# pathint/RankCompV3.jl

Hardware: AMD Instinct MI355X
Metric: gene-pair·sample comparisons/sec at 20k genes × 1k samples (higher is better)
Workload: dtype u16

## Files before the change

### rankcompv3.jl_amd/_ffi.py

```python
from __future__ import annotations

import ctypes
import os
import subprocess
from typing import NamedTuple

import numpy as np

_HERE = os.path.dirname(os.path.abspath(__file__))
LIB_PATH = os.environ.get("REO_LIB_PATH") or os.path.join(_HERE, "libreo_hip.so")
CSRC = os.path.join(_HERE, "csrc")

REO_OK, REO_EINVAL, REO_EHIP, REO_ECOMM, REO_ENOMEM = 0, -1, -2, -3, -4
NTIMINGS = 12
CALL_BINS = 8192

SYMBOLS = [
    "reo_version", "reo_last_error", "reo_create", "reo_destroy", "reo_trim_memory", "reo_set_shard", "reo_set_allreduce", "reo_set_allgather",
    "reo_create_multi", "reo_comm_unique_id", "reo_comm_init_rank",
    "reo_set_matrix_f64", "reo_set_matrix_i64", "reo_set_matrix_dev_f64", "reo_set_matrix_dev_i64",
    "reo_set_matrix_f32", "reo_set_matrix_i32", "reo_set_matrix_dev_f32", "reo_set_matrix_dev_i32",
    "reo_set_matrix_rm_f64", "reo_set_matrix_rm_i64", "reo_set_matrix_rm_f32", "reo_set_matrix_rm_i32",
    "reo_set_matrix_csc_f64", "reo_set_matrix_csc_i64", "reo_set_matrix_csc_f32", "reo_set_matrix_csc_i32",
    "reo_set_groups", "reo_compute_thresholds", "reo_set_thresholds", "reo_get_thresholds", "reo_threshold",
# ... 837 lines not shown
    def get_matrix(self) -> np.ndarray:
        info = self.info()
        dt = {1: np.float64, 2: np.int64, 3: np.float32}.get(info["resident_dtype"])
        if dt is None:
            raise DimensionMismatch(REO_EINVAL, "no expression matrix set")
        out = np.zeros((info["G"], info["S"]), dtype=dt, order="F")
        check(self._L.reo_get_matrix(self._h, _ptr(out), out.nbytes))
        return out

    def set_profiling(self, on: bool) -> None:
        check(self._L.reo_set_profiling(self._h, 1 if on else 0))

    def reset_timings(self) -> None:
        check(self._L.reo_reset_timings(self._h))

    def timings(self) -> dict:
        ms = np.zeros(NTIMINGS, dtype=np.float64)
        check(self._L.reo_get_timings(self._h, _ptr(ms), NTIMINGS))
        return {"transform_ms": ms[0], "k1_ms": ms[1], "k2_ms": ms[2], "iter_ms": ms[3], "k3_ms": max(ms[3] - ms[2], 0.0), "k2_launches": int(ms[4]),
                "k1_launches": int(ms[5]), "exchange_ms": ms[6], "pseudobulk_ms": ms[7], "k2_full_ms": ms[8],
                "k2_full_launches": int(ms[9]), "k2_delta_ms": ms[10], "set_matrix_host_wall_ms": ms[11]}

    def info(self) -> dict:
        w = np.zeros(32, dtype=np.int64)
        check(self._L.reo_get_info(self._h, _ptr(w), 32))
        v = np.zeros(28, dtype=np.int64)
        v[:] = w[:28]
        return {"G": int(v[0]), "S": int(v[1]), "Gp": int(v[2]), "table_bytes": int(v[3]), "has_ties": int(v[4]),
                "tiles_owned": int(v[5]), "tiles_total": int(v[6]), "tile_i": int(v[7]), "chunk_j": int(v[8]),
                "chunks_per_panel": int(v[9]), "unit_h": int(v[10]), "sample_slots": int(v[11]),
                "shared_group_counts": int(v[12]), "group_count_bytes": int(v[13]), "transform_in_lds": int(v[14]), "xcc_local_histograms": int(v[15]),
                "cycle_period": int(v[16]), "cycle_found_at_pass": int(v[17]), "cycle_passes_skipped": int(v[18]), "upload_link_bytes": int(v[19]),
                "eager_range_launches": int(v[20]), "rowmajor_upload": int(v[21]),
                "csc_upload": int(v[22]), "csc_nnz": int(v[23]), "resident_dtype": int(v[24]),
                "k1_slot_order": int(v[25]), "k1_half_tiles_separated": int(v[26]), "csc_device": int(v[27]),
                "k1_unslot_form": int(w[28]), "contrast_treat": int(w[29]), "k1_slot_sides": int(w[30]),
                "masked_build": int(w[31])}
```

### rankcompv3.jl_amd/csrc/api.hip

```cpp
#include <execinfo.h>
#include <signal.h>
#include <unistd.h>

#include <ctime>
#include <algorithm>
#include <chrono>
#include <cmath>
#include <cstdarg>
#include <cstdio>
#include <cstdlib>
#include <cstring>

#include "reo_internal.h"
#include "contrast.h"
#include "masked_pairs.h"
#include "sample_counts.h"
#include "upload_csc.h"

#include <mutex>
#include <unordered_map>

namespace reo {

static thread_local std::string g_err;
thread_local bool tl_release_synced = false;

namespace {
struct Block { void *p; size_t bytes; int device; bool pinned; };
struct Pool {
    std::mutex mu;
    std::vector<Block> free_blocks;
    std::unordered_map<void *, size_t> live;
    size_t cached = 0, cap = size_t(16384) << 20;
    bool read_env = false;
};
Pool &pool() { static Pool *p = new Pool(); return *p; }
// ... 569 lines not shown
    }
    REO_HIP_CHECK(hipSetDevice(device));
    reo_ctx *c = new (std::nothrow) reo_ctx();
    if (!c) { set_error("out of host memory"); return REO_ENOMEM; }
    c->device = device;
    c->seed = seed;
    if (const char *e = getenv("REO_K1_WAVE")) c->k1_wave = (e[0] != '0');
    if (const char *e = getenv("REO_K1_HALF")) c->k1_half = (e[0] != '0');
    if (const char *e = getenv("REO_K1_SLOTS")) c->k1_slots = (e[0] != '0');
    if (const char *e = getenv("REO_K1_QUEUE")) c->k1_queue = (e[0] != '0');
    if (const char *e = getenv("REO_K1_UNSLOT")) { const int v = atoi(e); c->k1_unslot = (v == 8 || v == 4) ? v : (e[0] == '0' ? 0 : -1); }
    if (const char *e = getenv("REO_K1_SLOT_SIDES")) { const int v = atoi(e); c->k1_slot_sides = (v == 1 || v == 2) ? v : 0; }
    if (const char *e = getenv("REO_K1_WORKERS")) c->k1_workers = std::max(1, atoi(e));
    if (const char *e = getenv("REO_K1_ORDER")) c->k1_order = std::max(0, std::min(2, atoi(e)));
    {
        int n = 0;
        if (hipDeviceGetAttribute(&n, hipDeviceAttributeMultiprocessorCount, c->device) == hipSuccess && n > 0) c->n_cus = n;
    }
    if (const char *e = getenv("REO_SPIN_WAIT")) c->spin_wait = (e[0] != '0');
    if (const char *e = getenv("REO_CHECK_HOOK_TABLE")) c->check_hook_table = (e[0] != '0');
    if (const char *e = getenv("REO_SHARE_GROUP_COUNTS")) c->share_counts = (e[0] != '0');
    if (const char *e = getenv("REO_LIGHT_BAND")) c->light_band = std::max(0, atoi(e));
    if (const char *e = getenv("REO_HIST_BELOW")) c->hist_below = std::max(0, atoi(e));
    if (const char *e = getenv("REO_CYCLE")) c->cycle_watch = atoi(e) != 0;
    if (const char *e = getenv("REO_LIGHT")) c->light_mode = e[0] == '0' ? 0 : (e[0] == '2' ? 2 : (e[0] == '3' ? 3 : 1));
    c->light_window = light_window(); c->light_min_g = light_min_genes();
    if (const char *e = getenv("REO_LIGHT_WINDOW")) c->light_window = std::max(1, std::min(31, atoi(e)));
    if (const char *e = getenv("REO_LIGHT_MIN_G")) c->light_min_g = std::max(64, atoi(e));
    if (const char *e = getenv("REO_STATE_MIRROR")) c->state_mirror_wanted = (e[0] != '0');
    if (const char *e = getenv("REO_EXCHANGE_WAVES")) c->x_waves = std::max(1, std::min(8, atoi(e)));
    if (const char *e = getenv("REO_EAGER_UPLOAD")) c->eager_mode = std::max(0, std::min(2, atoi(e)));
    if (const char *e = getenv("REO_EAGER_CHUNK")) c->eager_chunk = std::max(1, atoi(e));
    if (const char *e = getenv("REO_EAGER_GATE")) c->eager_gate = atoi(e) != 0;
    if (const char *e = getenv("REO_EAGER_RANGES")) c->eager_ranges = std::max(1, std::min(6, atoi(e)));
    if (const char *e = getenv("REO_UPLOAD_THREADS")) c->upload_threads = std::max(0, std::min(64, atoi(e)));
    c->debug_passes = getenv("REO_DEBUG_PASSES") != nullptr;
    c->debug_stamps = getenv("REO_DEBUG_STAMPS") != nullptr;
    c->k1_stamps = getenv("REO_K1_STAMPS") != nullptr;
    hipError_t e = handle_stream(&c->stream, 0);
    if (e != hipSuccess) { delete c; set_error("hipStreamCreate failed: %s", hipGetErrorString(e)); return REO_EHIP; }
    int ok = 0;
    const char *xe = getenv("REO_XCC_LOCAL");
    if (!(xe && xe[0] == '0')) {
        const int32_t rc = xcc_selftest(c, &ok);
        if (rc) { reo_destroy(c); return rc; }
    }
// ... 823 lines not shown
{
    if (!c) { set_error("null context"); return REO_EINVAL; }
    collect_timings(c);
    for (double &v : c->t_ms) v = 0.0;
    return REO_OK;
}

int32_t reo_get_timings(reo_ctx *c, double *ms, int32_t n)
{
    if (!c || !ms) { set_error("null argument"); return REO_EINVAL; }
    collect_timings(c);
    for (int i = 0; i < n && i < REO_NTIMINGS; ++i) ms[i] = c->t_ms[i];
    return REO_OK;
}

int32_t reo_get_info(reo_ctx *c, int64_t *info, int32_t n)
{
    if (!c || !info) { set_error("null argument"); return REO_EINVAL; }
    int64_t separated = 0;
    if (n > 26 && c->last_k1_slots) {
        int32_t rc = use(c);
        if (rc || (rc = launch_slot_separated(c, &separated))) return rc;
    }
    const int64_t v[32] = {c->G, c->S, c->Gp, static_cast<int64_t>(c->table.n * sizeof(uint32_t)), c->has_ties,
                           c->tiles_owned, c->tiles_total, kTileI, c->k1_cj, c->k1_q, kUnitH,
                           c->goff32.empty() ? 0 : c->goff32.back(), c->last_k1_shared,
                           static_cast<int64_t>(c->gcounts.n * sizeof(uint16_t)), c->transform_in_lds, c->xcc_local,
                           c->it_cycle_period, c->it_cycle_at, c->it_cycle_skipped, c->narrowed_bytes, c->eager_range_launches, c->rowmajor_upload,
                           c->csc_upload, c->csc_nnz, c->dtype, c->last_k1_slots, separated, c->csc_device,
                           c->last_k1_slots ? c->last_k1_unslot : 0, c->built_k >= 0 ? c->built_treat : -1,
                           c->last_k1_slots ? c->last_k1_slot_sides : 0, (c->built_k >= 0 && c->built_masked) ? 1 : 0};
    for (int i = 0; i < n && i < 32; ++i) info[i] = v[i];
    return REO_OK;
}

}
```

### rankcompv3.jl_amd/csrc/kernels.hip

```cpp
#include <algorithm>
#include <chrono>
#include <cstddef>
#include <cstdio>
#include <cstdlib>
#include <cstring>
#include <mutex>
#include <type_traits>

#include "reo_internal.h"
#include "k1_items.h"
#include "k1_slots.h"
#include "k1_queue.h"
#include "contrast.h"
#include "tie_coin.h"

namespace reo {

namespace {

template <bool COH, class T>
__device__ __forceinline__ T ldc(const T *p)
{
    if (COH) return __hip_atomic_load(p, __ATOMIC_RELAXED, __HIP_MEMORY_SCOPE_AGENT);
    return *p;
}
template <bool COH, class T>
__device__ __forceinline__ void stc(T *p, T v)
{
    if (COH) __hip_atomic_store(p, v, __ATOMIC_RELAXED, __HIP_MEMORY_SCOPE_AGENT);
    else *p = v;
}

// ... 1501 lines not shown
    int G, Gp, Wp;
    int n_iter, n_conv;
    int a0, b0;
    double pval_deg, padj_deg;
    uint32_t *refbits[2];
    uint8_t *refbytes[2];
    int32_t *raw;
    uint32_t *delta_list;
    double *result;
    double *chunk_v; uint16_t *chunk_i; double *chunk_spl;
    double *sorted_d; double *sorted_spl; double *sorted_p;
    uint32_t *rank_s; uint32_t *rank_a;
    double *part; double *blockmin; double *scal;
    int32_t *trace; int32_t *modes;
    double *cand;
    int32_t *hist;
    int hist_stride;
    int32_t *mrank;
    int replay;
    int k2_idx;
    int xcc_local;
    int32_t *olist;
    int hist_below;
    uint8_t *snap;
    int32_t *clist; int band;
    int window, light_min_g;
    unsigned long long *stamps;
    IterState *host_st;
};

#ifdef REO_STAMPS
#define STAMP(a, k) do { if (blockIdx.x == 0 && threadIdx.x == 0) (a).stamps[k] = __builtin_amdgcn_s_memrealtime(); } while (0)
#else
#define STAMP(a, k) do { } while (0)
#endif

__device__ __forceinline__ void raise_fault(const IterArgs &a, int code)
{
    a.st->fault = code;
    if (a.host_st) a.host_st->fault = code;
}

constexpr int kCandMax = 64;
constexpr int kWindow = 24;
constexpr int kLightMinG = 4096;

// ... 672 lines not shown
    const double n = n0 + n1 + n2;
    const double mean = (n0 * mean0 + n1 * mean1 + n2 * mean2) / n;
    const double m2 = (q0 + n0 * (mean0 - mean) * (mean0 - mean)) + (q1 + n1 * (mean1 - mean) * (mean1 - mean)) +
                      (q2 + n2 * (mean2 - mean) * (mean2 - mean));
    se = sqrt(m2 / (n - 1.0));
    return static_cast<int>(n) == a.b0 - a.a0 + 1;
}

template <bool COH>
__device__ __forceinline__ bool slice_std(const IterArgs &a, const double *cand, int npart, int below_a, int below_b, int cnt_a, int cnt_b,
                                          double (*sel)[4], double *red, double &se, double &va, double &vb)
{
    const int lane = threadIdx.x & 63, wave = threadIdx.x >> 6;
    double x = 0.0, pn[kPartPer] = {0.0}, pm[kPartPer] = {0.0}, pq[kPartPer] = {0.0};
    if (wave < 2 && lane < (wave ? cnt_b : cnt_a) && lane < kCandMax) x = ldc<COH>(cand + wave * kCandMax + lane);
#pragma unroll
    for (int u = 0; u < kPartPer; ++u) {
        const int w = threadIdx.x + 256 * u;
        if (w < npart) { pn[u] = ldc<COH>(a.part + 3 * w); pm[u] = ldc<COH>(a.part + 3 * w + 1); pq[u] = ldc<COH>(a.part + 3 * w + 2); }
    }
    return slice_std_vals(a, x, pn, pm, pq, below_a, below_b, cnt_a, cnt_b, sel, red, se, va, vb);
}

__device__ __forceinline__ int hist_first(int kstar, int below) { return kstar > below ? kstar - below : 0; }

template <int NT = 4>
__device__ __forceinline__ int bh_cut4(const int (&hv)[4][8], int G, int tile0, int &carry_io, int roff = 0)
{
    __shared__ __attribute__((aligned(16))) int wsum[4][4];
    __shared__ int wbest[4];
    const int lane = threadIdx.x & 63, wave = threadIdx.x >> 6;
    int s[4], inc[4];
#pragma unroll
    for (int e = 0; e < NT; ++e) {
        s[e] = ((hv[e][0] + hv[e][1]) + (hv[e][2] + hv[e][3])) + ((hv[e][4] + hv[e][5]) + (hv[e][6] + hv[e][7]));
        inc[e] = s[e];
    }
#pragma unroll
    for (int o = 1; o < 64; o <<= 1)
#pragma unroll
        for (int e = 0; e < NT; ++e)
        { const int u = __shfl_up(inc[e], o, 64); if (lane >= o) inc[e] += u; }
    if (lane == 63)
#pragma unroll
        for (int e = 0; e < NT; ++e) wsum[e][wave] = inc[e];
    lds_barrier();
    int best = 0, carry = carry_io;
#pragma unroll
    for (int e = 0; e < NT; ++e) {
        const int4 ws = *reinterpret_cast<const int4 *>(wsum[e]);
        int run = carry + inc[e] - s[e] + (wave > 0 ? ws.x : 0) + (wave > 1 ? ws.y : 0) + (wave > 2 ? ws.z : 0);
        const int r0 = roff + ((tile0 + e) * 256 + threadIdx.x) * 8 + 1;
#pragma unroll
        for (int u = 0; u < 8; ++u) { run += hv[e][u]; if (r0 + u <= G && run >= r0 + u) best = max(best, r0 + u); }
        carry += ws.x + ws.y + ws.z + ws.w;
    }
    carry_io = carry;
#pragma unroll
    for (int o = 32; o > 0; o >>= 1) { const int u = __shfl_xor(best, o, 64); best = u > best ? u : best; }
    if (lane == 0) wbest[wave] = best;
    lds_barrier();
    const int k = max(max(wbest[0], wbest[1]), max(wbest[2], wbest[3]));
    lds_barrier();
    return k;
}

template <int BYTES>
__device__ __forceinline__ void warm_kernargs()
{
    const uint32_t *ka = (const uint32_t *)__builtin_amdgcn_kernarg_segment_ptr();
    uint32_t t[(BYTES + 63) / 64];
#pragma unroll
    for (int q = 0; q < (BYTES + 63) / 64; ++q) t[q] = ka[16 * q];
#pragma unroll
    for (int q = 0; q < (BYTES + 63) / 64; ++q) asm volatile("" ::"s"(t[q]));
}

constexpr int kListPre = 5;
constexpr int kHeadPre = 20;

__device__ __forceinline__ int mrank_slot(int i) { return (i & ~255) + 4 * (i & 63) + ((i >> 6) & 3); }

__device__ __forceinline__ unsigned xcc_id()
{
    unsigned x;
    asm volatile("s_getreg_b32 %0, hwreg(HW_REG_XCC_ID, 0, 4)" : "=s"(x));
    return x & (kHistParts - 1);
// ... 64 lines not shown
    const bool crowded = reload_all || __ballot(nflag > 1) != 0;
    if (!crowded && __ballot(nflag == 1)) note_changes(nflag == 1, wave + 4 * selq, sel);
#pragma unroll 1
    for (int R = crowded ? wave : wave + 4 * kHeadPre; R < nrow; R += 4) note_changes(true, R, load_rank_row<COH>(mrank, R, lane));
}

template <bool TAIL, bool LIST>
__global__ __launch_bounds__(256) void kl_head(IterArgs a, LightState *ls, int b)
{
    const int G = a.G, Gp = a.Gp;
    const int i = blockIdx.x * 256 + threadIdx.x;
    const int lane = threadIdx.x & 63, wave = threadIdx.x >> 6;
    __shared__ uint32_t dl[kDeltaMax];
    __shared__ int s_n, s_nn, s_fb;
    __shared__ uint4 dbuf[kDeltaMax * 8];
    __shared__ double red[256];
    warm_kernargs<sizeof(IterArgs) + 16>();
    if (!TAIL) STAMP(a, 8);
    const int pb = (b - 1) & 1;
    LightRec r;
    int bfail = 0, sig = 0, nlow = 0, cdiff = 0, cfound = 0;
    int hv[4][8];
    int4 hx[kHistParts][2];
    int4 mv[kHeadPre];
    int2 le[kListPre];
    int lcnt[kListPre];
    int own_m = 0;
    int4 r0 = make_int4(0, 0, 0, 0), r1 = make_int4(0, 0, 0, 0);
    double win[4];
    uint32_t cyc_w[kDeltaMax / 64];
    uint8_t cyc_s[kDeltaMax / 64];
    int cyc_open = 0;
    bool cyc_renew = false;
    const int nrow = (G + 255) >> 8;
    if (b > 0) {
        const int32_t *hist = a.hist + static_cast<size_t>(pb) * kHistParts * a.hist_stride;
#pragma unroll
        for (int e = 0; e < 4; ++e)
#pragma unroll
            for (int u = 0; u < 8; ++u) hv[e][u] = 0;
#pragma unroll
        for (int x = 0; x < kHistParts; ++x) {
            const int4 *hp = reinterpret_cast<const int4 *>(hist + static_cast<size_t>(x) * a.hist_stride + threadIdx.x * 8);
            hx[x][0] = hp[0]; hx[x][1] = hp[1];
        }
#pragma unroll
        for (int q = 0; q < kHeadPre; ++q) {
            const int R = wave + 4 * q;
            mv[q] = make_int4(0, 0, 0, 0);
            if (!LIST && R < nrow) mv[q] = reinterpret_cast<const int4 *>(a.mrank)[R * 64 + lane];
        }
        if (LIST) {
            const int32_t *cl = a.clist + static_cast<size_t>(pb) * kListStride;
#pragma unroll
            for (int q = 0; q < kListPre; ++q) {
                const int e = threadIdx.x + 256 * q, blk = e / kListCap;
                le[q] = make_int2(0, 0); lcnt[q] = 0;
                if (blk < nrow) { lcnt[q] = cl[blk]; le[q] = reinterpret_cast<const int2 *>(cl + kListWgs)[e]; }
            }
        }
        if (i < G) own_m = a.mrank[mrank_slot(i)];
    }
    if (!TAIL && i < G) {
        const int4 *o = reinterpret_cast<const int4 *>(a.raw + static_cast<size_t>(i) * kRaw);
        r0 = o[0]; r1 = o[1];
    }
    if (b > 0) {
        const LightSlot *ps = &ls->slot[b - 1];
        r = ps->rec; bfail = ps->bfail; cdiff = ps->cdiff; cfound = ps->cfound;
#pragma unroll
        for (int q = 0; q < kSpread; ++q) { sig += ps->lc.sig[q][0]; nlow += ps->lc.nlow[q][0]; }
#pragma unroll
        for (int q = 0; q < 4; ++q) win[q] = ps->wnext[q];
    } else {
#pragma unroll
        for (int q = 0; q < 4; ++q) win[q] = a.scal[1 + q];
    }
    if (!TAIL) STAMP(a, 0);
    int n = 0;
    bool inref = false;
    bool stepped = false;
    if (b == 0) {
        const IterState *st = a.st;
        r.t = st->passes; r.nref = st->nref; r.nref_prev = st->nref_prev; r.done = st->done; r.need_full = st->need_full;
        r.raw_pass = st->raw_pass; r.ran = 0; r.dcnt = st->delta_cnt[r.t & 1]; r.kstar = -1;
        r.cper = st->cyc_period; r.cpow = st->cyc_pow; r.clam = st->cyc_lam; r.csel = st->cyc_sel; cdiff = st->cyc_ndiff;
        r.active = (!r.done && r.t < a.n_iter && !r.need_full) ? 1 : 0;
        if (r.active) {
            n = r.raw_pass == r.t ? 0 : min(r.dcnt, kDeltaMax);
            if (static_cast<int>(threadIdx.x) < n) dl[threadIdx.x] = a.delta_list[static_cast<size_t>(r.t & 1) * Gp + threadIdx.x];
            inref = i < G && a.refbytes[r.t & 1][i] != 0;
            lds_barrier();
        }
    } else if (r.active && bfail) {
        r.active = 0; r.need_full = 1;
    } else if (r.active && cfound) {
        r.active = 0; r.cper = cfound;
    } else if (r.active) {
        const int t = r.t, cur = t & 1, nxt = cur ^ 1;
        const int off = hist_first(r.kstar, a.hist_below), srel = sig - off;
        {
            const int32_t *hist = a.hist + static_cast<size_t>(pb) * kHistParts * a.hist_stride;
#pragma unroll
            for (int x = 0; x < kHistParts; ++x) {
                hv[0][0] += hx[x][0].x; hv[0][1] += hx[x][0].y; hv[0][2] += hx[x][0].z; hv[0][3] += hx[x][0].w;
                hv[0][4] += hx[x][1].x; hv[0][5] += hx[x][1].y; hv[0][6] += hx[x][1].z; hv[0][7] += hx[x][1].w;
            }
            if (srel > 2048) {
#pragma unroll 1
                for (int x = 0; x < kHistParts; ++x)
#pragma unroll
                    for (int e = 1; e < 4; ++e) {
                        const int4 *hp = reinterpret_cast<const int4 *>(hist + static_cast<size_t>(x) * a.hist_stride + (e * 256 + threadIdx.x) * 8);
                        const int4 h0 = hp[0], h1 = hp[1];
                        hv[e][0] += h0.x; hv[e][1] += h0.y; hv[e][2] += h0.z; hv[e][3] += h0.w; hv[e][4] += h1.x; hv[e][5] += h1.y; hv[e][6] += h1.z; hv[e][7] += h1.w;
                    }
            }
        }
        int carry = nlow;
        int kstar = srel > 2048 ? bh_cut4(hv, G, 0, carry, off) : bh_cut4<1>(hv, G, 0, carry, off);
        if (srel > 8192) {
            const int32_t *hist = a.hist + static_cast<size_t>(pb) * kHistParts * a.hist_stride;
            const int ntile = (min(G - off, srel) + 2047) / 2048;
#pragma unroll 1
            for (int tile0 = 4; tile0 < ntile; tile0 += 4) {
#pragma unroll
                for (int e = 0; e < 4; ++e)
#pragma unroll
                    for (int u = 0; u < 8; ++u) hv[e][u] = 0;
#pragma unroll 1
                for (int x = 0; x < kHistParts; ++x)
#pragma unroll
                    for (int e = 0; e < 4; ++e) {
                        if ((tile0 + e) * 2048 >= a.hist_stride) continue;
                        const int4 *hp = reinterpret_cast<const int4 *>(hist + static_cast<size_t>(x) * a.hist_stride + ((tile0 + e) * 256 + threadIdx.x) * 8);
                        const int4 h0 = hp[0], h1 = hp[1];
                        hv[e][0] += h0.x; hv[e][1] += h0.y; hv[e][2] += h0.z; hv[e][3] += h0.w; hv[e][4] += h1.x; hv[e][5] += h1.y; hv[e][6] += h1.z; hv[e][7] += h1.w;
                    }
                kstar = max(kstar, bh_cut4(hv, G, tile0, carry, off));
            }
        }
        const bool cut_lost = off > 0 && kstar == 0;
        if (!TAIL) STAMP(a, 1);
        if (cut_lost) {
            r.active = 0; r.need_full = 1;
        } else {
        if (threadIdx.x == 0) { s_n = 0; s_nn = 0; s_fb = 0; }
        lds_barrier();
        if (LIST) {
            const uint32_t base = static_cast<uint32_t>(kstar) + 1u;
            bool bad = r.kstar < 0 || kstar < r.kstar - a.band || kstar > r.kstar + a.band;
            auto note = [&](int cnt, int2 ent, int e) {
                bad = bad || cnt > kListCap;
                const bool chd = (e % kListCap) < cnt && static_cast<int>(static_cast<uint32_t>(ent.x) - base) >= 0;
                const unsigned long long cm = __ballot(chd);
                if (cm) {
                    const uint32_t nb = (static_cast<uint32_t>(ent.x) >> 31) ^ 1u;
                    const unsigned long long am = __ballot(chd && nb);
                    int pos = 0;
                    if (lane == 0) { pos = atomicAdd(&s_n, __popcll(cm)); atomicAdd(&s_nn, 2 * __popcll(am) - __popcll(cm)); }
                    pos = __shfl(pos, 0, 64);
                    const int at = pos + __popcll(cm & ((1ULL << lane) - 1ULL));
                    if (chd && at < kDeltaMax) dl[at] = (static_cast<uint32_t>(ent.y) << 1) | nb;
                }
            };
#pragma unroll
            for (int q = 0; q < kListPre; ++q) note(lcnt[q], le[q], threadIdx.x + 256 * q);
            const int32_t *cl = a.clist + static_cast<size_t>(pb) * kListStride;
// ... 62 lines not shown
            for (int o = 32; o > 0; o >>= 1) d += __shfl_xor(d, o, 64);
            cdiff += d;
            cfound = cdiff == 0 ? cyc_open : 0;
        } else if (cyc_open < 0) {
            cdiff = 0x40000000; cfound = 0;
        } else {
            cfound = stepped ? 0 : cfound;
        }
        if (cyc_renew) cdiff = 0;
    };
    if (TAIL) {
        if (blockIdx.x == 0 && wave == 0) {
            cyc_close();
            if (cfound) r.cper = cfound;
        }
        if (blockIdx.x == 0 && threadIdx.x == 0) {
            IterState *st = a.st;
            st->cyc_period = r.cper; st->cyc_pow = r.cpow; st->cyc_lam = r.clam; st->cyc_sel = r.csel; st->cyc_ndiff = cdiff;
            st->passes = r.t; st->nref = r.nref; st->nref_prev = r.nref_prev; st->done = r.done; st->need_full = r.need_full;
            st->i_iter = r.t - (r.done ? 1 : 0);
            st->raw_pass = r.raw_pass;
            st->delta_cnt[r.t & 1] = r.dcnt;
            if (r.ran) st->last_full = 0;
            if (stepped) { a.scal[1] = win[0]; a.scal[2] = win[1]; a.scal[3] = win[2]; a.scal[4] = win[3]; }
            if (a.host_st) {
                IterState *h = a.host_st;
                h->passes = r.t; h->done = r.done; h->need_full = r.need_full; h->delta_cnt[r.t & 1] = r.dcnt;
                h->cyc_period = r.cper;
                if (r.ran) h->last_full = 0;
            }
        }
        return;
    }
    if (r.active) r.raw_pass = r.t;
    if (blockIdx.x == 0 && threadIdx.x == 0) ls->slot[b].rec = r;
    if (!r.active || static_cast<int>(blockIdx.x) * 256 >= G) {
        if (blockIdx.x == 0 && wave == 0) { cyc_close(); if (lane == 0) { ls->slot[b].cdiff = cdiff; ls->slot[b].cfound = cfound; } }
        return;
    }
    const int pbuf = b & 1;
    LightCnt *lc = &ls->slot[b].lc;
    const double wa_lo = win[0], wa_hi = win[1], wb_lo = win[2], wb_hi = win[3];
    double v = 0.0;
    bool inner = false, inA = false, inB = false, belowA = false, belowB = false;
    if (n) {
        int d[kRaw];
        delta_counts_block(a.table, a.Wp, dl, n, d, dbuf);
        if (!TAIL) STAMP(a, 3);
        if (i < G) {
            r0.x += d[0]; r0.y += d[1]; r0.z += d[2]; r0.w += d[3];
            r1.x += d[4]; r1.y += d[5]; r1.z += d[6]; r1.w += d[7];
            int4 *o = reinterpret_cast<int4 *>(a.raw + static_cast<size_t>(i) * kRaw);
            o[0] = r0; o[1] = r1;
        }
    }
    if (i < G) {
        int32_t c[9];
        const bool tok = tallies_from(r0, r1, r.nref - (inref ? 1 : 0), c);
        double out[5] = {1.0, 0.0, 0.0, 0.0, 0.0};
        if (tok) mccullagh3<false>(c, out);
        v = out[1];
        if (!tok || !(fabs(v) < INFINITY)) { v = 0.0; raise_fault(a, kFaultTallies); }
        if (!TAIL) STAMP(a, 4);
        a.result[11 * static_cast<size_t>(G) + i] = v;
#pragma unroll
        for (int x = 0; x < kHistParts; ++x) a.hist[(static_cast<size_t>(pbuf) * kHistParts + x) * a.hist_stride + i] = 0;
        belowA = v < wa_lo; inA = !belowA && v <= wa_hi;
        belowB = v < wb_lo; inB = !belowB && v <= wb_hi;
        inner = v > wa_hi && v < wb_lo;
    }
    if (!TAIL) STAMP(a, 5);
    if (G <= 65535) {
        const double nb = static_cast<double>(__popcll(__ballot(inner))), sum = wave_sum(inner ? v : 0.0);
        const double mean = nb > 0.0 ? sum / nb : 0.0;
        const double m2 = wave_sum(inner ? (v - mean) * (v - mean) : 0.0);
        if (lane == 0) { double *pp = a.part + 3 * (4 * blockIdx.x + wave); pp[0] = nb; pp[1] = mean; pp[2] = m2; }
    } else {
        double nb, sum;
        block_sum2_256(inner ? 1.0 : 0.0, inner ? v : 0.0, red, nb, sum);
        const double mean = nb > 0.0 ? sum / nb : 0.0;
        const double m2 = block_sum_256(inner ? (v - mean) * (v - mean) : 0.0, red);
        if (threadIdx.x == 0) { a.part[3 * blockIdx.x] = nb; a.part[3 * blockIdx.x + 1] = mean; a.part[3 * blockIdx.x + 2] = m2; }
    }
    if (!TAIL) STAMP(a, 6);
    const unsigned long long mA = __ballot(inA), mB = __ballot(inB), bA = __ballot(belowA), bB = __ballot(belowB);
    int baseA = 0, baseB = 0;
    if (lane == 0) {
        if (mA) baseA = atomicAdd(&lc->cnt_a, __popcll(mA));
        if (mB) baseB = atomicAdd(&lc->cnt_b, __popcll(mB));
        if (bA) spread_add(lc->below_a, __popcll(bA), a.xcc_local);
        if (bB) spread_add(lc->below_b, __popcll(bB), a.xcc_local);
    }
// ... 31 lines not shown
    const double wd0 = a.scal[5], wd1 = a.scal[6], wd2 = a.scal[7], wd3 = a.scal[8];
    const double d1 = live ? a.result[11 * static_cast<size_t>(G) + i] : 0.0;
    const uint8_t ob_e = live ? a.refbytes[0][i] : 0, ob_o = live ? a.refbytes[1][i] : 0;
    if (!active) return;
    STAMP(a, 20);
    __shared__ double sel[3][4];
    double se = 0.0, va = 0.0, vb = 0.0;
    bool ok = slice_std_split(a, x, pn, pm, pq, below_a, below_b, cnt_a, cnt_b, sel, se, va, vb);
    ok = ok && (va + wd1 < vb - wd2);
    STAMP(a, 21);
    if (blockIdx.x == 0 && threadIdx.x == 0) {
        if (ok) {
            a.scal[0] = se;
            sl->wnext[0] = va - wd0; sl->wnext[1] = va + wd1; sl->wnext[2] = vb - wd2; sl->wnext[3] = vb + wd3;
        } else {
            sl->bfail = 1;
        }
    }
    if (!ok) return;
    const double p = live ? normal_p(d1, se) : 1.0;
    if (live) a.result[i] = p;
    const int m = live ? bh_rank(p, G, a.padj_deg) : G + 1;
    STAMP(a, 22);
    {
        const int off = hist_first(rec_kstar, a.hist_below);
        const unsigned long long first = __ballot(m == 1 && off == 0), finite = __ballot(m <= G), low = __ballot(m <= off);
        const bool lead1 = m == 1 && off == 0 && lane == __ffsll(static_cast<long long>(first)) - 1;
        const bool binned = m > off && m <= G && !(m == 1 && off == 0);
        if (a.xcc_local) {
            int32_t *hist = a.hist + (static_cast<size_t>(pbuf) * kHistParts + xcc_id()) * a.hist_stride;
            if (lead1) __hip_atomic_fetch_add(&hist[0], __popcll(first), __ATOMIC_RELAXED, __HIP_MEMORY_SCOPE_WORKGROUP);
            else if (binned) __hip_atomic_fetch_add(&hist[m - 1 - off], 1, __ATOMIC_RELAXED, __HIP_MEMORY_SCOPE_WORKGROUP);
        } else {
            int32_t *hist = a.hist + static_cast<size_t>(pbuf) * kHistParts * a.hist_stride;
            if (lead1) atomicAdd(&hist[0], __popcll(first));
            else if (binned) atomicAdd(&hist[m - 1 - off], 1);
        }
        if (lane == 0 && finite) spread_add(lc->sig, __popcll(finite), a.xcc_local);
        if (lane == 0 && low) spread_add(lc->nlow, __popcll(low), a.xcc_local);
    }
    {
        __shared__ int32_t row[256];
        const uint32_t oldbit = ((rec_t & 1) ? ob_o : ob_e) != 0 ? 0x80000000u : 0u;
        row[4 * lane + wave] = live ? static_cast<int32_t>(static_cast<uint32_t>(p <= a.pval_deg ? m : G + 2) | oldbit) : 0;
        lds_barrier();
        a.mrank[blockIdx.x * 256 + threadIdx.x] = row[threadIdx.x];
    }
    if (rec_kstar >= 0) {
        __shared__ int s_c;
        if (threadIdx.x == 0) s_c = 0;
        lds_barrier();
        const int kp = rec_kstar, rk = p <= a.pval_deg ? m : G + 2;
        const bool ob = ((rec_t & 1) ? ob_o : ob_e) != 0;
        const bool want = live && ((rk > kp - a.band && rk <= kp + a.band) || (rk > kp + a.band && !ob) || (rk <= kp - a.band && ob));
        const unsigned long long cm = __ballot(want);
        int pos = 0;
        if (cm && lane == 0) pos = atomicAdd(&s_c, __popcll(cm));
        pos = __shfl(pos, 0, 64) + __popcll(cm & ((1ULL << lane) - 1ULL));
        int32_t *cl = a.clist + static_cast<size_t>(pbuf) * kListStride;
        if (want && pos < kListCap)
            reinterpret_cast<int2 *>(cl + kListWgs)[blockIdx.x * kListCap + pos] = make_int2(static_cast<int>(static_cast<uint32_t>(rk) | (ob ? 0x80000000u : 0u)), i);
        lds_barrier();
        if (threadIdx.x == 0) cl[blockIdx.x] = min(s_c, kListCap + 1);
    }
    STAMP(a, 23);
}

constexpr double kEtaMin = 1.0 / 2048.0, kEtaMax = 1.0 / 64.0, kEta0 = 1.0 / 128.0;

// ... 1356 lines not shown
    k3_tallies<<<(G + 255) / 256, 256, 0, c->stream>>>(c->raw.p, c->refbytes[0].p, nref, G, c->cont.p);
    REO_HIP_CHECK(hipGetLastError());
    return REO_OK;
}

static IterArgs iter_args(reo_ctx *c, int replay)
{
    IterArgs a;
    a.st = c->state.p; a.table = c->table.p;
    a.G = static_cast<int>(c->G); a.Gp = c->Gp; a.Wp = c->Wp;
    a.n_iter = c->it_n_iter; a.n_conv = c->it_n_conv; a.a0 = c->it_a0; a.b0 = c->it_b0;
    a.pval_deg = c->it_pval_deg; a.padj_deg = c->it_padj_deg;
    for (int t = 0; t < 2; ++t) { a.refbits[t] = c->refbits[t].p; a.refbytes[t] = c->refbytes[t].p; }
    a.raw = c->raw.p; a.delta_list = c->delta_list.p; a.result = c->result.p;
    const int nchunk = (a.G + kSortChunk - 1) / kSortChunk;
    a.chunk_v = c->chunk_v.p; a.chunk_i = c->chunk_i.p;
    a.chunk_spl = c->chunk_v.p + static_cast<size_t>(nchunk) * kSortChunk;
    a.sorted_d = c->sorted_d.p; a.sorted_spl = c->sorted_d.p + ((c->G + 63) / 64) * 64;
    a.sorted_p = c->sorted_p.p; a.rank_s = c->rank_s.p; a.rank_a = c->rank_a.p;
    a.part = c->part.p; a.blockmin = c->blockmin.p; a.scal = c->scal.p;
    a.trace = c->trace.p; a.modes = nullptr;
    a.cand = c->cand.p; a.hist = c->hist.p; a.hist_stride = static_cast<int>(c->hist.n / (3 * kHistParts)); a.mrank = c->mrank.p;
    a.replay = replay; a.k2_idx = 0;
    a.clist = c->clist.p; a.olist = c->olist.p; a.band = c->light_band; a.hist_below = c->hist_below; a.snap = c->snap.p; a.xcc_local = c->xcc_local;
    a.window = c->light_window; a.light_min_g = (c->it_no_light || c->light_mode == 0) ? 0x7FFFFFFF : c->light_min_g;
    a.stamps = reinterpret_cast<unsigned long long *>(c->scal.p + 32);
    a.host_st = c->state_mirror ? c->host_state : nullptr;
    return a;
}

int32_t launch_full_pass(reo_ctx *c, bool replay)
{
    IterArgs a = iter_args(c, replay ? 1 : 0);
    const int G = a.G, nb = (G + 255) / 256;
    const int nchunk = (G + kSortChunk - 1) / kSortChunk;
    const int nmerge = (nchunk * kSortChunk + kMergeThreads / kMergeLanes - 1) / (kMergeThreads / kMergeLanes);
    if (!replay) {
        if (c->k2_idx < static_cast<int>(c->modes.n)) { a.modes = c->modes.p; a.k2_idx = c->k2_idx; }
        ++c->k2_idx;
        tic(c, 2);
        k2_tally<<<(G + 3) / 4, 256, 0, c->stream>>>(a);
        toc(c);
        c->t_ms[4] += 1.0;
    }
    k3_derive<<<nb, 256, 0, c->stream>>>(a);
    k3_sort_chunks<<<nchunk, kSortChunk, 0, c->stream>>>(a);
    const size_t spl_bytes = static_cast<size_t>(nchunk) * kSplit * sizeof(double);
// ... 91 lines not shown
```

### rankcompv3.jl_amd/csrc/reo_internal.h

```cpp
#pragma once

#include <hip/hip_runtime.h>

#include <cstdint>
#include <functional>
#include <string>
#include <vector>

#include "reo_hip.h"

namespace reo {

constexpr int kTileJ = 256;
constexpr int kTileI = 32;
constexpr int kPlanes = 4;
constexpr int kUnitH = 32;
constexpr int kRJ = 4;
constexpr int kRJTies = 2;
constexpr int kMaxGenes = 262143;
constexpr int kGenePad = 1024;
constexpr int kRaw = 8;
constexpr int kDeltaMax = 128;
constexpr int kSortChunk = 1024;

struct IterState {
    int32_t done;
    int32_t passes;
    int32_t nref;
    int32_t i_iter;
    int32_t ticket;
    int32_t nn_acc;
    int32_t delta_cnt[2];
    int32_t need_full;
    int32_t raw_pass;
    int32_t nref_prev;
    int32_t last_full;
    int32_t fault;
    int32_t kstar;
    int32_t kcut_acc;
    int32_t cyc_period;
    int32_t cyc_pow;
    int32_t cyc_lam;
    int32_t cyc_sel;
    int32_t cyc_ndiff;
    int32_t pad[4];
};
constexpr int kFaultBarrier = 1;
constexpr int kFaultTallies = 2;

constexpr int kLightBatch = 128;
struct LightRec {
    int32_t active;
    int32_t t;
    int32_t nref, nref_prev, done, need_full, raw_pass;
    int32_t ran;
    int32_t dcnt;
    int32_t kstar;
    int32_t cper, cpow, clam, csel;
};
constexpr int kHistParts = 8;
constexpr int kSpread = 8;
constexpr int kListCap = 16;
constexpr int kListWgs = 1024;
static_assert(kMaxGenes <= kListWgs * 256, "the light passes' lists and block moments (clist, part) hold kListWgs workgroups of 256 genes");
constexpr int kPartPer = kListWgs / 256;
constexpr int kListStride = kListWgs + kListWgs * kListCap * 2;
constexpr int kOneListCap = 16;
constexpr int kOneListMax = 512;
constexpr int kOneStride = 256 + 256 * kOneListCap * 4;
struct LightCnt {
    int32_t cnt_a, cnt_b;
    int32_t pad[30];
    int32_t below_a[kSpread][32];
    int32_t below_b[kSpread][32];
    int32_t sig[kSpread][32];
    int32_t nsure[kSpread][32];
    int32_t nlow[kSpread][32];
};
struct LightSlot {
    LightRec rec;
    int32_t bfail;
    int32_t cdiff;
    int32_t cfound;
    int32_t pad0[5];
    double wnext[4];
    double se_base;
    double eta;
    double pad1[15];
    LightCnt lc;
};
struct LightState { LightSlot slot[kLightBatch + 2]; };
static_assert(sizeof(LightSlot) % 128 == 0, "LightSlot layout");

void set_error(const char *fmt, ...);

#define REO_HIP_CHECK(expr)                                                              \
    do {                                                                                 \
        hipError_t e_ = (expr);                                                          \
        if (e_ != hipSuccess) {                                                          \
            ::reo::set_error("%s failed: %s (%s:%d)", #expr, hipGetErrorString(e_),      \
                             __FILE__, __LINE__);                                        \
            return e_ == hipErrorOutOfMemory ? REO_ENOMEM : REO_EHIP;                    \
        }                                                                                \
    } while (0)

hipError_t pool_alloc(void **p, size_t bytes, bool pinned);
void pool_free(void *p, size_t bytes, bool pinned);
extern thread_local bool tl_release_synced;
hipError_t handle_stream(hipStream_t *s, int kind);
hipError_t handle_event(hipEvent_t *e, int kind);
void release_stream(hipStream_t s, int kind);
// ... 173 lines not shown
    reo::DevBuf<uint32_t> delta_list;
    reo::DevBuf<int32_t> cont;
    reo::DevBuf<double> result;
    reo::DevBuf<double> sorted_d;
    reo::DevBuf<double> sorted_p;
    reo::DevBuf<uint32_t> rank_s, rank_a;
    reo::DevBuf<double> scal;
    reo::DevBuf<double> blockmin;
    reo::DevBuf<double> chunk_v;
    reo::DevBuf<uint16_t> chunk_i;
    reo::DevBuf<double> part;
    reo::DevBuf<reo::IterState> state;
    reo::DevBuf<int32_t> trace;
    reo::DevBuf<int32_t> modes;
    reo::DevBuf<double> cand;
    reo::DevBuf<unsigned> gridbar;
    reo::DevBuf<reo::LightState> lstate;
    reo::DevBuf<int32_t> clist;
    int light_band = 32;
    bool cycle_watch = true;
    reo::DevBuf<uint8_t> snap;
    int it_cycle_period = 0, it_cycle_at = 0, it_cycle_skipped = 0;
    int hist_below = 256;
    int xcc_local = 0;
    int light_window = 24, light_min_g = 4096;
    int light_mode = 1;
    reo::DevBuf<int32_t> olist;
    reo::DevBuf<int32_t> hist, mrank;
    double it_pval_deg = 1.0, it_padj_deg = 0.05;
    int it_n_iter = 0, it_n_conv = 0, it_a0 = 0, it_b0 = 0;
    int k2_idx = 0;
    int it_light_form = 1;
    bool it_no_light = false;
    reo::IterState *host_state = nullptr;
    bool state_mirror_wanted = true;
    bool debug_passes = false, debug_stamps = false, k1_stamps = false;
    bool state_mirror = false;
    uint8_t *host_ref = nullptr;
    size_t host_ref_cap = 0;

    bool profiling = false;
    double t_ms[REO_NTIMINGS] = {0};
    std::vector<std::pair<int, reo::StageTimer>> pending;
    std::vector<reo::StageTimer> pool;
    std::vector<size_t> open;
    std::vector<int32_t> k2_modes;
// ... 112 lines not shown
```

Baseline: 51390 billion.

## Bound light-pass BH cut histogram to a band with geometric overflow buckets

In the list-mode light iteration, the Benjamini-Hochberg cut histogram is limited to a fixed band of bins around the previous cut (below plus above) with 32 geometrically growing overflow buckets. The cut is found by one block-wide scan instead of tiled multi-pass scans over the whole gene range, and only the band words are cleared each pass instead of every gene's entry. When the overflow buckets cannot rule out a cut beyond the band, the pass is marked undecided and falls back to a full pass, which adds a counter and extra fallback work in exchange.

```diff
diff --git a/rankcompv3.jl_amd/_ffi.py b/rankcompv3.jl_amd/_ffi.py
--- a/rankcompv3.jl_amd/_ffi.py
+++ b/rankcompv3.jl_amd/_ffi.py
@@ -883,8 +883,8 @@
                 "k2_full_launches": int(ms[9]), "k2_delta_ms": ms[10], "set_matrix_host_wall_ms": ms[11]}
 
     def info(self) -> dict:
-        w = np.zeros(32, dtype=np.int64)
-        check(self._L.reo_get_info(self._h, _ptr(w), 32))
+        w = np.zeros(33, dtype=np.int64)
+        check(self._L.reo_get_info(self._h, _ptr(w), 33))
         v = np.zeros(28, dtype=np.int64)
         v[:] = w[:28]
         return {"G": int(v[0]), "S": int(v[1]), "Gp": int(v[2]), "table_bytes": int(v[3]), "has_ties": int(v[4]),
@@ -896,4 +896,4 @@
                 "csc_upload": int(v[22]), "csc_nnz": int(v[23]), "resident_dtype": int(v[24]),
                 "k1_slot_order": int(v[25]), "k1_half_tiles_separated": int(v[26]), "csc_device": int(v[27]),
                 "k1_unslot_form": int(w[28]), "contrast_treat": int(w[29]), "k1_slot_sides": int(w[30]),
-                "masked_build": int(w[31])}
+                "masked_build": int(w[31]), "band_cut_undecided": int(w[32])}
diff --git a/rankcompv3.jl_amd/csrc/api.hip b/rankcompv3.jl_amd/csrc/api.hip
--- a/rankcompv3.jl_amd/csrc/api.hip
+++ b/rankcompv3.jl_amd/csrc/api.hip
@@ -12,6 +12,7 @@
 #include <cstring>
 
 #include "reo_internal.h"
+#include "band_cut.h"
 #include "contrast.h"
 #include "masked_pairs.h"
 #include "sample_counts.h"
@@ -627,6 +628,9 @@
     if (const char *e = getenv("REO_SHARE_GROUP_COUNTS")) c->share_counts = (e[0] != '0');
     if (const char *e = getenv("REO_LIGHT_BAND")) c->light_band = std::max(0, atoi(e));
     if (const char *e = getenv("REO_HIST_BELOW")) c->hist_below = std::max(0, atoi(e));
+    if (const char *e = getenv("REO_HIST_ABOVE")) c->hist_above = std::max(0, atoi(e));
+    c->hist_below = std::min(c->hist_below, kBandBins);
+    c->hist_above = std::min(c->hist_above, kBandBins - c->hist_below);
     if (const char *e = getenv("REO_CYCLE")) c->cycle_watch = atoi(e) != 0;
     if (const char *e = getenv("REO_LIGHT")) c->light_mode = e[0] == '0' ? 0 : (e[0] == '2' ? 2 : (e[0] == '3' ? 3 : 1));
     c->light_window = light_window(); c->light_min_g = light_min_genes();
@@ -1496,16 +1500,17 @@
         int32_t rc = use(c);
         if (rc || (rc = launch_slot_separated(c, &separated))) return rc;
     }
-    const int64_t v[32] = {c->G, c->S, c->Gp, static_cast<int64_t>(c->table.n * sizeof(uint32_t)), c->has_ties,
+    const int64_t v[33] = {c->G, c->S, c->Gp, static_cast<int64_t>(c->table.n * sizeof(uint32_t)), c->has_ties,
                            c->tiles_owned, c->tiles_total, kTileI, c->k1_cj, c->k1_q, kUnitH,
                            c->goff32.empty() ? 0 : c->goff32.back(), c->last_k1_shared,
                            static_cast<int64_t>(c->gcounts.n * sizeof(uint16_t)), c->transform_in_lds, c->xcc_local,
                            c->it_cycle_period, c->it_cycle_at, c->it_cycle_skipped, c->narrowed_bytes, c->eager_range_launches, c->rowmajor_upload,
                            c->csc_upload, c->csc_nnz, c->dtype, c->last_k1_slots, separated, c->csc_device,
                            c->last_k1_slots ? c->last_k1_unslot : 0, c->built_k >= 0 ? c->built_treat : -1,
-                           c->last_k1_slots ? c->last_k1_slot_sides : 0, (c->built_k >= 0 && c->built_masked) ? 1 : 0};
-    for (int i = 0; i < n && i < 32; ++i) info[i] = v[i];
-    return REO_OK;
-}
-
-}
+                           c->last_k1_slots ? c->last_k1_slot_sides : 0, (c->built_k >= 0 && c->built_masked) ? 1 : 0,
+                           c->host_state ? c->host_state->band_undecided : 0};
+    for (int i = 0; i < n && i < 33; ++i) info[i] = v[i];
+    return REO_OK;
+}
+
+}
diff --git a/rankcompv3.jl_amd/csrc/band_cut.h b/rankcompv3.jl_amd/csrc/band_cut.h
--- /dev/null
+++ b/rankcompv3.jl_amd/csrc/band_cut.h
@@ -0,0 +1,67 @@
+#pragma once
+
+#include <cstdint>
+
+#if defined(__HIPCC__)
+#define REO_BC_FN __host__ __device__ inline
+#else
+#define REO_BC_FN inline
+#endif
+
+namespace reo {
+
+constexpr int kBandBins = 512;
+constexpr int kBandBuckets = 32;
+constexpr int kBandUndecided = -1;
+constexpr int kBandLost = -2;
+
+REO_BC_FN int band_first(int kstar, int below) { return kstar > below ? kstar - below : 0; }
+
+REO_BC_FN int band_top(int G, int off, int nbins)
+{
+    const int64_t t = static_cast<int64_t>(off) + nbins;
+    return t < G ? static_cast<int>(t) : G;
+}
+
+REO_BC_FN int band_unit(int nbins) { return nbins > 0 ? nbins : 1; }
+
+REO_BC_FN int band_edge(int G, int top, int w, int q)
+{
+    const int64_t e = static_cast<int64_t>(top) + static_cast<int64_t>(w) * ((int64_t(1) << q) - 1);
+    return e < G ? static_cast<int>(e) : G;
+}
+
+REO_BC_FN int band_bucket(int m, int top, int w)
+{
+    const uint32_t c = static_cast<uint32_t>((static_cast<int64_t>(m) - top + w - 1) / w);
+    return 32 - __builtin_clz(c);
+}
+
+REO_BC_FN int band_nbuckets(int G, int top, int w) { return top < G ? band_bucket(G, top, w) : 0; }
+
+REO_BC_FN int band_word(int m, int G, int off, int top, int nbins, int w)
+{
+    if (m <= off) return -1;
+    if (m > G) return -2;
+    if (m <= top) return m - 1 - off;
+    return nbins + band_bucket(m, top, w) - 1;
+}
+
+REO_BC_FN int band_cut_decide(const int32_t *bins, const int32_t *buckets, int nlow, int G, int off, int top, int w)
+{
+    int64_t run = nlow;
+    int best = 0;
+    for (int r = off + 1; r <= top; ++r) {
+        run += bins[r - off - 1];
+        if (run >= r) best = r;
+    }
+    const int Q = band_nbuckets(G, top, w);
+    for (int q = 1; q <= Q; ++q) {
+        run += buckets[q - 1];
+        if (run > band_edge(G, top, w, q - 1)) return kBandUndecided;
+    }
+    if (off > 0 && best == 0) return kBandLost;
+    return best;
+}
+
+}
diff --git a/rankcompv3.jl_amd/csrc/kernels.hip b/rankcompv3.jl_amd/csrc/kernels.hip
--- a/rankcompv3.jl_amd/csrc/kernels.hip
+++ b/rankcompv3.jl_amd/csrc/kernels.hip
@@ -8,6 +8,7 @@
 #include <type_traits>
 
 #include "reo_internal.h"
+#include "band_cut.h"
 #include "k1_items.h"
 #include "k1_slots.h"
 #include "k1_queue.h"
@@ -1555,6 +1556,7 @@
     int xcc_local;
     int32_t *olist;
     int hist_below;
+    int hist_above;
     uint8_t *snap;
     int32_t *clist; int band;
     int window, light_min_g;
@@ -2273,7 +2275,7 @@
     return slice_std_vals(a, x, pn, pm, pq, below_a, below_b, cnt_a, cnt_b, sel, red, se, va, vb);
 }
 
-__device__ __forceinline__ int hist_first(int kstar, int below) { return kstar > below ? kstar - below : 0; }
+__device__ __forceinline__ int hist_first(int kstar, int below) { return band_first(kstar, below); }
 
 template <int NT = 4>
 __device__ __forceinline__ int bh_cut4(const int (&hv)[4][8], int G, int tile0, int &carry_io, int roff = 0)
@@ -2314,6 +2316,38 @@
     const int k = max(max(wbest[0], wbest[1]), max(wbest[2], wbest[3]));
     lds_barrier();
     return k;
+}
+
+__device__ __forceinline__ int bh_cut_band(int c0, int c1, int bq, int nlow, int G, int off, int top, int w)
+{
+    __shared__ __attribute__((aligned(16))) int bsum[4];
+    __shared__ int bbest[4];
+    const int lane = threadIdx.x & 63, wave = threadIdx.x >> 6;
+    const int s = c0 + c1;
+    int inc = s, binc = lane < kBandBuckets ? bq : 0;
+#pragma unroll
+    for (int o = 1; o < 64; o <<= 1) {
+        const int u = __shfl_up(inc, o, 64), v = __shfl_up(binc, o, 64);
+        if (lane >= o) { inc += u; binc += v; }
+    }
+    if (lane == 63) bsum[wave] = inc;
+    lds_barrier();
+    const int4 ws = *reinterpret_cast<const int4 *>(bsum);
+    int run = nlow + inc - s + (wave > 0 ? ws.x : 0) + (wave > 1 ? ws.y : 0) + (wave > 2 ? ws.z : 0);
+    const int r0 = off + 2 * static_cast<int>(threadIdx.x) + 1;
+    int best = 0;
+    run += c0; if (r0 <= top && run >= r0) best = r0;
+    run += c1; if (r0 + 1 <= top && run >= r0 + 1) best = r0 + 1;
+    const int htop = nlow + ws.x + ws.y + ws.z + ws.w;
+    const int eprev = band_edge(G, top, w, lane < 31 ? lane : 31);
+    const bool broken = lane < 31 && eprev < G && htop + binc > eprev;
+    const bool undecided = __ballot(broken) != 0;
+#pragma unroll
+    for (int o = 32; o > 0; o >>= 1) { const int u = __shfl_xor(best, o, 64); best = u > best ? u : best; }
+    if (lane == 0) bbest[wave] = best;
+    lds_barrier();
+    const int k = max(max(bbest[0], bbest[1]), max(bbest[2], bbest[3]));
+    return undecided ? kBandUndecided : k;
 }
 
 template <int BYTES>
@@ -2424,6 +2458,9 @@
     int bfail = 0, sig = 0, nlow = 0, cdiff = 0, cfound = 0;
     int hv[4][8];
     int4 hx[kHistParts][2];
+    int2 bx[kHistParts];
+    int bqx[kHistParts];
+    int und = 0;
     int4 mv[kHeadPre];
     int2 le[kListPre];
     int lcnt[kListPre];
@@ -2437,14 +2474,24 @@
     const int nrow = (G + 255) >> 8;
     if (b > 0) {
         const int32_t *hist = a.hist + static_cast<size_t>(pb) * kHistParts * a.hist_stride;
-#pragma unroll
-        for (int e = 0; e < 4; ++e)
-#pragma unroll
-            for (int u = 0; u < 8; ++u) hv[e][u] = 0;
-#pragma unroll
-        for (int x = 0; x < kHistParts; ++x) {
-            const int4 *hp = reinterpret_cast<const int4 *>(hist + static_cast<size_t>(x) * a.hist_stride + threadIdx.x * 8);
-            hx[x][0] = hp[0]; hx[x][1] = hp[1];
+        if (LIST) {
+            const int nbins = a.hist_below + a.hist_above;
+#pragma unroll
+            for (int x = 0; x < kHistParts; ++x) {
+                const int32_t *hp = hist + static_cast<size_t>(x) * a.hist_stride;
+                bx[x] = reinterpret_cast<const int2 *>(hp)[threadIdx.x];
+                bqx[x] = hp[nbins + (lane & (kBandBuckets - 1))];
+            }
+        } else {
+#pragma unroll
+            for (int e = 0; e < 4; ++e)
+#pragma unroll
+                for (int u = 0; u < 8; ++u) hv[e][u] = 0;
+#pragma unroll
+            for (int x = 0; x < kHistParts; ++x) {
+                const int4 *hp = reinterpret_cast<const int4 *>(hist + static_cast<size_t>(x) * a.hist_stride + threadIdx.x * 8);
+                hx[x][0] = hp[0]; hx[x][1] = hp[1];
+            }
         }
 #pragma unroll
         for (int q = 0; q < kHeadPre; ++q) {
@@ -2469,7 +2516,7 @@
     }
     if (b > 0) {
         const LightSlot *ps = &ls->slot[b - 1];
-        r = ps->rec; bfail = ps->bfail; cdiff = ps->cdiff; cfound = ps->cfound;
+        r = ps->rec; bfail = ps->bfail; cdiff = ps->cdiff; cfound = ps->cfound; und = ps->und;
 #pragma unroll
         for (int q = 0; q < kSpread; ++q) { sig += ps->lc.sig[q][0]; nlow += ps->lc.nlow[q][0]; }
 #pragma unroll
@@ -2501,6 +2548,18 @@
     } else if (r.active) {
         const int t = r.t, cur = t & 1, nxt = cur ^ 1;
         const int off = hist_first(r.kstar, a.hist_below), srel = sig - off;
+        int kstar = 0;
+        bool undecided = false;
+        if (LIST) {
+            const int nbins = a.hist_below + a.hist_above;
+            int c0 = 0, c1 = 0, bq = 0;
+#pragma unroll
+            for (int x = 0; x < kHistParts; ++x) { c0 += bx[x].x; c1 += bx[x].y; bq += bqx[x]; }
+            c0 = 2 * static_cast<int>(threadIdx.x) < nbins ? c0 : 0;
+            c1 = 2 * static_cast<int>(threadIdx.x) + 1 < nbins ? c1 : 0;
+            kstar = bh_cut_band(c0, c1, bq, nlow, G, off, band_top(G, off, nbins), band_unit(nbins));
+            if (kstar == kBandUndecided) { undecided = true; kstar = 0; }
+        } else {
         {
             const int32_t *hist = a.hist + static_cast<size_t>(pb) * kHistParts * a.hist_stride;
 #pragma unroll
@@ -2520,7 +2579,7 @@
             }
         }
         int carry = nlow;
-        int kstar = srel > 2048 ? bh_cut4(hv, G, 0, carry, off) : bh_cut4<1>(hv, G, 0, carry, off);
+        kstar = srel > 2048 ? bh_cut4(hv, G, 0, carry, off) : bh_cut4<1>(hv, G, 0, carry, off);
         if (srel > 8192) {
             const int32_t *hist = a.hist + static_cast<size_t>(pb) * kHistParts * a.hist_stride;
             const int ntile = (min(G - off, srel) + 2047) / 2048;
@@ -2542,10 +2601,12 @@
                 kstar = max(kstar, bh_cut4(hv, G, tile0, carry, off));
             }
         }
+        }
         const bool cut_lost = off > 0 && kstar == 0;
         if (!TAIL) STAMP(a, 1);
-        if (cut_lost) {
+        if (cut_lost || undecided) {
             r.active = 0; r.need_full = 1;
+            und += undecided ? 1 : 0;
         } else {
         if (threadIdx.x == 0) { s_n = 0; s_nn = 0; s_fb = 0; }
         lds_barrier();
@@ -2654,18 +2715,20 @@
             st->raw_pass = r.raw_pass;
             st->delta_cnt[r.t & 1] = r.dcnt;
             if (r.ran) st->last_full = 0;
+            const int und_call = st->band_undecided + und;
+            st->band_undecided = und_call;
             if (stepped) { a.scal[1] = win[0]; a.scal[2] = win[1]; a.scal[3] = win[2]; a.scal[4] = win[3]; }
             if (a.host_st) {
                 IterState *h = a.host_st;
                 h->passes = r.t; h->done = r.done; h->need_full = r.need_full; h->delta_cnt[r.t & 1] = r.dcnt;
-                h->cyc_period = r.cper;
+                h->cyc_period = r.cper; h->band_undecided = und_call;
                 if (r.ran) h->last_full = 0;
             }
         }
         return;
     }
     if (r.active) r.raw_pass = r.t;
-    if (blockIdx.x == 0 && threadIdx.x == 0) ls->slot[b].rec = r;
+    if (blockIdx.x == 0 && threadIdx.x == 0) { ls->slot[b].rec = r; ls->slot[b].und = und; }
     if (!r.active || static_cast<int>(blockIdx.x) * 256 >= G) {
         if (blockIdx.x == 0 && wave == 0) { cyc_close(); if (lane == 0) { ls->slot[b].cdiff = cdiff; ls->slot[b].cfound = cfound; } }
         return;
@@ -2695,11 +2758,18 @@
         if (!tok || !(fabs(v) < INFINITY)) { v = 0.0; raise_fault(a, kFaultTallies); }
         if (!TAIL) STAMP(a, 4);
         a.result[11 * static_cast<size_t>(G) + i] = v;
-#pragma unroll
-        for (int x = 0; x < kHistParts; ++x) a.hist[(static_cast<size_t>(pbuf) * kHistParts + x) * a.hist_stride + i] = 0;
+        if (b == 0) {
+#pragma unroll
+            for (int x = 0; x < kHistParts; ++x) a.hist[(static_cast<size_t>(pbuf) * kHistParts + x) * a.hist_stride + i] = 0;
+        }
         belowA = v < wa_lo; inA = !belowA && v <= wa_hi;
         belowB = v < wb_lo; inB = !belowB && v <= wb_hi;
         inner = v > wa_hi && v < wb_lo;
+    }
+    if (b > 0) {
+        const int nword = (a.hist_below + a.hist_above + kBandBuckets) * kHistParts, nthr = ((G + 255) >> 8) * 256;
+        for (int j = i; j < nword; j += nthr)
+            a.hist[(static_cast<size_t>(pbuf) * kHistParts + (j & (kHistParts - 1))) * a.hist_stride + (j >> 3)] = 0;
     }
     if (!TAIL) STAMP(a, 5);
     if (G <= 65535) {
@@ -2777,19 +2847,32 @@
     if (live) a.result[i] = p;
     const int m = live ? bh_rank(p, G, a.padj_deg) : G + 1;
     STAMP(a, 22);
+    const int off = hist_first(rec_kstar, a.hist_below);
+    const bool bandf = rec_kstar >= 0;
+    const int nbins = a.hist_below + a.hist_above, top = bandf ? band_top(G, off, nbins) : G;
+    int32_t *const hist = a.hist + (static_cast<size_t>(pbuf) * kHistParts + (a.xcc_local ? xcc_id() : 0u)) * a.hist_stride;
+    __shared__ int s_bk[4][kBandBuckets];
+    int nq = 0;
     {
-        const int off = hist_first(rec_kstar, a.hist_below);
         const unsigned long long first = __ballot(m == 1 && off == 0), finite = __ballot(m <= G), low = __ballot(m <= off);
-        const bool lead1 = m == 1 && off == 0 && lane == __ffsll(static_cast<long long>(first)) - 1;
-        const bool binned = m > off && m <= G && !(m == 1 && off == 0);
+        const bool lead1 = m == 1 && off == 0 && top >= 1 && lane == __ffsll(static_cast<long long>(first)) - 1;
+        const bool binned = m > off && m <= top && !(m == 1 && off == 0);
         if (a.xcc_local) {
-            int32_t *hist = a.hist + (static_cast<size_t>(pbuf) * kHistParts + xcc_id()) * a.hist_stride;
             if (lead1) __hip_atomic_fetch_add(&hist[0], __popcll(first), __ATOMIC_RELAXED, __HIP_MEMORY_SCOPE_WORKGROUP);
             else if (binned) __hip_atomic_fetch_add(&hist[m - 1 - off], 1, __ATOMIC_RELAXED, __HIP_MEMORY_SCOPE_WORKGROUP);
         } else {
-            int32_t *hist = a.hist + static_cast<size_t>(pbuf) * kHistParts * a.hist_stride;
             if (lead1) atomicAdd(&hist[0], __popcll(first));
             else if (binned) atomicAdd(&hist[m - 1 - off], 1);
+        }
+        if (bandf) {
+            const int w = band_unit(nbins);
+            int lo = top;
+            for (int q = 1; lo < G; ++q) {
+                const int hi = band_edge(G, top, w, q);
+                const unsigned long long in = __ballot(m > lo && m <= hi);
+                if (lane == 0) s_bk[wave][q - 1] = __popcll(in);
+                lo = hi; nq = q;
+            }
         }
         if (lane == 0 && finite) spread_add(lc->sig, __popcll(finite), a.xcc_local);
         if (lane == 0 && low) spread_add(lc->nlow, __popcll(low), a.xcc_local);
@@ -2800,6 +2883,13 @@
         row[4 * lane + wave] = live ? static_cast<int32_t>(static_cast<uint32_t>(p <= a.pval_deg ? m : G + 2) | oldbit) : 0;
         lds_barrier();
         a.mrank[blockIdx.x * 256 + threadIdx.x] = row[threadIdx.x];
+        if (static_cast<int>(threadIdx.x) < nq) {
+            const int t = threadIdx.x, cnt = (s_bk[0][t] + s_bk[1][t]) + (s_bk[2][t] + s_bk[3][t]);
+            if (cnt) {
+                if (a.xcc_local) __hip_atomic_fetch_add(&hist[nbins + t], cnt, __ATOMIC_RELAXED, __HIP_MEMORY_SCOPE_WORKGROUP);
+                else atomicAdd(&hist[nbins + t], cnt);
+            }
+        }
     }
     if (rec_kstar >= 0) {
         __shared__ int s_c;
@@ -4202,7 +4292,7 @@
     a.trace = c->trace.p; a.modes = nullptr;
     a.cand = c->cand.p; a.hist = c->hist.p; a.hist_stride = static_cast<int>(c->hist.n / (3 * kHistParts)); a.mrank = c->mrank.p;
     a.replay = replay; a.k2_idx = 0;
-    a.clist = c->clist.p; a.olist = c->olist.p; a.band = c->light_band; a.hist_below = c->hist_below; a.snap = c->snap.p; a.xcc_local = c->xcc_local;
+    a.clist = c->clist.p; a.olist = c->olist.p; a.band = c->light_band; a.hist_below = c->hist_below; a.hist_above = c->hist_above; a.snap = c->snap.p; a.xcc_local = c->xcc_local;
     a.window = c->light_window; a.light_min_g = (c->it_no_light || c->light_mode == 0) ? 0x7FFFFFFF : c->light_min_g;
     a.stamps = reinterpret_cast<unsigned long long *>(c->scal.p + 32);
     a.host_st = c->state_mirror ? c->host_state : nullptr;
diff --git a/rankcompv3.jl_amd/csrc/reo_internal.h b/rankcompv3.jl_amd/csrc/reo_internal.h
--- a/rankcompv3.jl_amd/csrc/reo_internal.h
+++ b/rankcompv3.jl_amd/csrc/reo_internal.h
@@ -43,7 +43,8 @@
     int32_t cyc_lam;
     int32_t cyc_sel;
     int32_t cyc_ndiff;
-    int32_t pad[4];
+    int32_t band_undecided;
+    int32_t pad[3];
 };
 constexpr int kFaultBarrier = 1;
 constexpr int kFaultTallies = 2;
@@ -83,10 +84,11 @@
     int32_t cdiff;
     int32_t cfound;
     int32_t pad0[5];
+    int32_t und;
     double wnext[4];
     double se_base;
     double eta;
-    double pad1[15];
+    double pad1[14];
     LightCnt lc;
 };
 struct LightState { LightSlot slot[kLightBatch + 2]; };
@@ -306,6 +308,7 @@
     reo::DevBuf<uint8_t> snap;
     int it_cycle_period = 0, it_cycle_at = 0, it_cycle_skipped = 0;
     int hist_below = 256;
+    int hist_above = 256;
     int xcc_local = 0;
     int light_window = 24, light_min_g = 4096;
     int light_mode = 1;
```

After: 50980 billion. Within noise of the previous version (-0.8%).
